# DarioSamo/sm64rt-legacy-renderer

Hardware: AMD Instinct MI355X
Metric: Mrays/s (primary+shadow), sample scene 1080p 1spp (higher is better)
Workload: dtype f32

## Files before the change

sm64rt-legacy-renderer_amd/csrc/kernels.h:

```cpp
#pragma once
#include <hip/hip_runtime.h>
#include "rt64_gpu.h"

#define LBVH_SMALL_MAX 4096u
enum { LBVH_MODE_TRIANGLES = 0, LBVH_MODE_INSTANCES = 1 };

struct LbvhArgs {
    int mode, refit;
    uint32_t n;
    const uint8_t *vertices; uint32_t vertexStride; const uint32_t *indices;
    const GpuInstance *instances;
    GpuNode *nodes;
    GpuTri *tris;
    BlasHeader *header;
    uint32_t *sortedIndex, *morton, *leafParent;
    void *scratch; size_t scratchBytes;
};

size_t lbvh_small_lds_bytes(uint32_t n);
size_t lbvh_large_scratch_bytes(uint32_t n);
hipError_t lbvh_launch(const LbvhArgs &args, hipStream_t stream);
hipError_t lbvh_launch_large(const LbvhArgs &args, hipStream_t stream);
hipError_t lbvh_launch_batch(const LbvhArgs *deviceArgs, uint32_t count, uint32_t maxN, hipStream_t stream);

hipError_t tile_texture_launch(const uint8_t *rgba, uint32_t *tiled, uint32_t width, uint32_t height, hipStream_t stream);
hipError_t bc7_decode_launch(const uint8_t *blocks, uint8_t *rgba, uint32_t width, uint32_t height, hipStream_t stream);

#define RT_CACHE_MAX_WORDS 1536
#define RT_STACK_LDS 24
#define RT_STACK_LDS_CACHED 16
#define RT_STACK_SPILL 84
#define RT_STACK_SPILL_HEADER 2
hipError_t launch_stack_slab_init(uint32_t *slab, size_t lanes, const uint32_t *flagDevicePointer, hipStream_t s);
#define RT_GRID_BLOCKS 2048
#define RT_TIMING_WAVES ((8192u + 8u) * 4u)
#define RT_MAX_BOUNCE_GROUPS 65536u
#define RT_MAX_FRAME_GROUPS 8192u
size_t rt_stack_spill_bytes(int width, int rows);

hipError_t launch_scene_cache_image(const GpuInstance *instances, const uint32_t *tlasIndex, const GpuNode *tlasNodes, uint32_t cacheInstances, void *image, bool blasOnly, hipStream_t s);
hipError_t launch_primary_trace(const FrameParams &P, const ViewImages &I, int32_t *hitInstance, bool klist, hipStream_t s);
hipError_t launch_primary_shade(const FrameParams &P, const ViewImages &I, const int32_t *hitInstance, int cur, bool transparentLighting, bool lean, hipStream_t s);
hipError_t launch_direct(const FrameParams &P, const ViewImages &I, int cur, bool lean, hipStream_t s);
enum { BOUNCE_WALK_PLAIN = 0, BOUNCE_WALK_REFILL = 1, BOUNCE_WALK_SPLIT = 2 };
hipError_t launch_indirect(const FrameParams &P, const ViewImages &I, int cur, bool writeFiltered, bool klist, int walk, unsigned groups, int writeGuide, hipStream_t s);
hipError_t launch_indirect_constant(const FrameParams &P, const ViewImages &I, int cur, hipStream_t s);
hipError_t launch_refraction(const FrameParams &P, const ViewImages &I, bool klist, hipStream_t s);
hipError_t launch_reflection(const FrameParams &P, const ViewImages &I, bool klist, int pass, bool last, int parity, hipStream_t s);
hipError_t launch_gaussian(const uint16_t *in, uint16_t *out, int width, int height, int y0, int y1, hipStream_t s);
hipError_t launch_compose_post(const FrameParams &P, const ViewImages &I, int cur, bool lean, bool writeFinal, hipStream_t s);
hipError_t launch_lean_frame(const FrameParams &P, const ViewImages &I, int32_t *hitInstance, int cur, bool full, int ownedY0, int ownedY1, unsigned maxGroups, bool perWave, hipStream_t s);
hipError_t launch_post_process(const FrameParams &P, const ViewImages &I, hipStream_t s);
hipError_t launch_primary_shade_simple(const FrameParams &P, const ViewImages &I, const int32_t *hitInstance, int cur, bool transparentLighting, bool lean, hipStream_t s);
hipError_t launch_direct_simple(const FrameParams &P, const ViewImages &I, int cur, bool lean, hipStream_t s);
hipError_t launch_indirect_simple(const FrameParams &P, const ViewImages &I, int cur, bool writeFiltered, bool klist, int walk, unsigned groups, int writeGuide, hipStream_t s);
hipError_t launch_refraction_simple(const FrameParams &P, const ViewImages &I, bool klist, hipStream_t s);
// ... 37 lines not shown
```

sm64rt-legacy-renderer_amd/csrc/lbvh.hip:

```cpp
#include <algorithm>
#include "kernels.h"
#include "device_math.h"

#define LBVH_THREADS 1024
#define LBVH_COUNTING_MAX 1024u

namespace {

DEV uint32_t float_to_ordered(float f) { uint32_t u = __float_as_uint(f); return (u & 0x80000000u) ? ~u : (u | 0x80000000u); }
DEV float ordered_to_float(uint32_t u) { return __uint_as_float((u & 0x80000000u) ? (u & 0x7FFFFFFFu) : ~u); }

DEV uint32_t morton30(uint32_t x, uint32_t y, uint32_t z) {
    uint32_t v[3] = { x & 1023u, y & 1023u, z & 1023u };
    uint32_t code = 0;
#pragma unroll
    for (int k = 0; k < 3; k++) {
        uint32_t t = v[k];
        t = (t | (t << 16)) & 0x030000FFu;
        t = (t | (t << 8)) & 0x0300F00Fu;
        t = (t | (t << 4)) & 0x030C30C3u;
        t = (t | (t << 2)) & 0x09249249u;
        code |= t << k;
    }
    return code;
// ... 578 lines not shown

hipError_t lbvh_launch_large(const LbvhArgs &args, hipStream_t stream) {
    if (!args.scratch || args.scratchBytes < lbvh_large_scratch_bytes(args.n)) return hipErrorInvalidValue;
    const uint32_t n = args.n;
    LargeScratch L = carve(args.scratch, n);
    const uint32_t grid = std::min<uint32_t>((n + LG_THREADS - 1) / LG_THREADS, 2048u);
    if (!args.refit) {
        hipLaunchKernelGGL(lg_init_bounds, dim3(1), dim3(64), 0, stream, L.bounds);
        hipLaunchKernelGGL(lg_bounds_kernel, dim3(grid), dim3(LG_THREADS), 0, stream, args, L.bounds);
        hipLaunchKernelGGL(lg_morton_kernel, dim3(grid), dim3(LG_THREADS), 0, stream, args, L.bounds, L.keyA, L.valA);
        uint32_t *kin = L.keyA, *vin = L.valA, *kout = L.keyB, *vout = L.valB;
        for (int shift = 0; shift < 32; shift += 8) {
            hipLaunchKernelGGL(lg_hist_kernel, dim3(L.blocks), dim3(LG_THREADS), 0, stream, kin, n, shift, L.hist, L.blocks);
            hipLaunchKernelGGL(lg_scan_rows_kernel, dim3(256), dim3(LG_THREADS), 0, stream, L.hist, L.blocks);
            hipLaunchKernelGGL(lg_scatter_kernel, dim3(L.blocks), dim3(LG_THREADS), 0, stream, kin, vin, kout, vout, n, shift, L.hist, L.blocks);
            std::swap(kin, kout); std::swap(vin, vout);
        }
        hipLaunchKernelGGL(lg_karras_kernel, dim3(grid), dim3(LG_THREADS), 0, stream, args, kin, vin);
    }
    hipLaunchKernelGGL(lg_leaves_kernel, dim3(grid), dim3(LG_THREADS), 0, stream, args, L.leafBox, L.done);
    uint32_t lists = (n + LG_CHUNK - 1) / LG_CHUNK;
    uint32_t *inList = L.rootList, *inCount = L.rootCount;
    hipLaunchKernelGGL(lg_fit_local_kernel, dim3(lists), dim3(LG_FIT_THREADS), 0, stream, args, L.leafBox, L.nodeBox, inList, inCount);
    for (uint64_t granule = (uint64_t)LG_CHUNK * LG_FAN;; granule *= LG_FAN) {
        const uint32_t groups = (lists + LG_FAN - 1) / LG_FAN;
        uint32_t *outList = inList + (size_t)lists * LG_ROOT_SLOTS, *outCount = inCount + lists;
        hipLaunchKernelGGL(lg_fit_group_kernel, dim3(groups), dim3(1024), 0, stream, args, L.leafBox, L.nodeBox, L.done, inList, inCount, lists,
                           groups == 1 ? 0xFFFFFFFFu : (uint32_t)granule, outList, outCount);
        if (groups == 1) break;
        lists = groups; inList = outList; inCount = outCount;
    }
    return hipGetLastError();
}
```

sm64rt-legacy-renderer_amd/csrc/rt64_gpu.h:

```cpp
#pragma once
#include <stdint.h>
#include "../../include/rt64.h"

#define RT64_LEAF_BIT 0x80000000u
#define RT64_NO_CHILD 0xFFFFFFFFu
#define RT64_MAX_MIPS 16
#define RT64_MAX_LIGHTS 16
#define RT64_MAX_HIT_QUERIES 16

struct alignas(16) GpuNode {
    float lmin[3], lmax[3];
    float rmin[3], rmax[3];
    uint32_t left, right, parent, pad;
};
static_assert(sizeof(GpuNode) == 64, "GpuNode");

struct alignas(16) GpuTri {
    float v0[3]; uint32_t prim;
    float v1[3]; uint32_t pad1;
    float v2[3]; uint32_t pad2;
};
static_assert(sizeof(GpuTri) == 48, "GpuTri");
#define GPU_TRI_FETCH_SLACK_BYTES (sizeof(GpuNode) - sizeof(GpuTri))
static_assert(GPU_TRI_FETCH_SLACK_BYTES == 16 && GPU_TRI_FETCH_SLACK_BYTES <= sizeof(GpuTri), "a triangle is fetched as one node-sized record");
inline size_t gpu_tri_array_bytes(size_t triangles) { return triangles * sizeof(GpuTri) + GPU_TRI_FETCH_SLACK_BYTES; }

struct BlasHeader {
    float bmin[3]; uint32_t count;
    float bmax[3]; uint32_t depth;
};

struct GpuTexture {
    const uint8_t *texels;
    uint32_t width, height, mips, pow2;
    uint32_t mipOffset[RT64_MAX_MIPS];
};

struct GpuCombiner {
    int8_t c[2][4];
    int8_t inputCount, useTex0, useTex1, vertexUV;
    int8_t doSingle[2], doMultiply[2], doMix[2];
    int8_t colorAlphaSame, optAlpha, optTextureEdge, optNoise;
    int16_t vertexSize, normalOffset, uvOffset, inputOffset[4];
};

enum : uint32_t {
    GPU_INST_CULL_DISABLE = 1u << 0,
    GPU_INST_OPAQUE       = 1u << 1,
    GPU_INST_NORMAL_MAP   = 1u << 2,
    GPU_INST_SPECULAR_MAP = 1u << 3,
    GPU_INST_SHADOW_OPAQUE = 1u << 4,
};

struct alignas(16) GpuInstance {
    float objectToWorld[16];
    float objectToWorldNormal[16];
    float objectToWorldPrevious[16];
    float worldToObject[16];
    const GpuNode *nodes;
    const GpuTri *tris;
    const uint8_t *vertices;
    const uint32_t *indices;
    const BlasHeader *header;
    RT64_MATERIAL material;
    GpuCombiner cc;
    int32_t texDiffuse, texNormal, texSpecular;
    uint32_t filter, hAddr, vAddr;
    uint32_t flags;
    uint32_t triCount;
    uint32_t meshVersion;
    uint32_t cacheNodeOffset;
};

struct alignas(16) GpuRasterInstance {
    const uint8_t *vertices;
    const uint32_t *indices;
    uint32_t vertexStride, triCount;
    uint32_t firstTri;
    GpuCombiner cc;
    int32_t texDiffuse;
    uint32_t filter, hAddr, vAddr;
    int32_t scissorRect[4], viewportRect[4];
    uint32_t meshVersion;
    uint32_t texSerial;
};

struct FrameParams {
    float view[16], viewI[16], prevViewI[16], projection[16], projectionI[16], viewProj[16], prevViewProj[16];
    float cameraU[4], cameraV[4], cameraW[4];
    float viewport[4], resolution[4];
    float ambientBaseColor[4], ambientNoGIColor[4], eyeLightDiffuseColor[4], eyeLightSpecularColor[4];
    float skyDiffuseMultiplier[4], skyHSLModifier[4];
    float pixelJitter[2];
    float skyYawOffset, giDiffuseStrength, giSkyStrength, motionBlurStrength;
    int32_t skyPlaneTexIndex;
// ... 33 lines not shown
struct ViewImages {
    uint16_t *viewDirection;
    float *shadingPosition;
    uint16_t *shadingNormal, *shadingSpecular;
    uint8_t *diffuse;
    int32_t *instanceId, *firstInstanceId;
    uint16_t *directLight[2], *indirectLight[2], *filteredDirect[2], *filteredIndirect[2];
    uint16_t *reflection, *refraction, *transparent;
    uint16_t *flow;
    uint8_t *reactiveMask, *lockMask;
    uint16_t *normal[2];
    float *depth[2];
    float *output;
    uint8_t *final;
    uint32_t *primaryHit;
    float *moments[2];
    uint4 *bounceRecords;
    uint32_t *bounceLists, *bounceCounts;
    BounceRadiance *bounceResults;
    uint4 *svgfGuide;
    uint32_t *svgfYoung;
    uint4 *reflState0, *reflState1; uint32_t *reflTag;
    uint32_t *reflectFlags;
    uint4 *klistA;
    uint2 *klistB;
    uint32_t *klistCount;
};

#if defined(__HIPCC__)
#define RT64_HD __host__ __device__ inline
#else
#define RT64_HD inline
#endif
#define RT64_GATHER_MAX_RANKS 64
struct GatherLayout { int height, count, mode; int starts[RT64_GATHER_MAX_RANKS + 1]; };
RT64_HD int gather_band_rows(int height, int count) { return (height + count - 1) / count; }
RT64_HD int gather_row_owner(const GatherLayout &L, int y, int *packed) {
    if (L.count <= 1) { *packed = y; return 0; }
    if (L.mode == 2) { int r = 0; while (r + 1 < L.count && y >= L.starts[r + 1]) r++; *packed = y - L.starts[r]; return r; }
    if (L.mode == 1) { const int b = gather_band_rows(L.height, L.count); *packed = y % b; return y / b; }
    const int strip = y / 16;
    *packed = (strip / L.count) * 16 + (y & 15);
    return strip % L.count;
}
RT64_HD int gather_owned_rows(const GatherLayout &L, int rank) {
    if (L.count <= 1) return L.height;
    if (L.mode == 2) return L.starts[rank + 1] - L.starts[rank];
    if (L.mode == 1) { const int b = gather_band_rows(L.height, L.count), y0 = rank * b, y1 = (rank + 1) * b; return (y1 < L.height ? y1 : L.height) - (y0 < L.height ? y0 : L.height); }
    int rows = 0;
    for (int y = rank * 16; y < L.height; y += L.count * 16) rows += (y + 16 <= L.height ? 16 : L.height - y);
    return rows;
}
RT64_HD int gather_max_owned_rows(const GatherLayout &L) {
    if (L.mode == 2) { int m = 0; for (int r = 0; r < L.count; r++) { const int n = L.starts[r + 1] - L.starts[r]; m = n > m ? n : m; } return m; }
    return L.mode == 1 ? gather_band_rows(L.height, L.count) : (((L.height + 15) / 16 + L.count - 1) / L.count) * 16;
}
RT64_HD GatherLayout gather_layout(int height, int count, int mode) { GatherLayout L; L.height = height; L.count = count < 1 ? 1 : count; L.mode = mode; for (int i = 0; i <= RT64_GATHER_MAX_RANKS; i++) L.starts[i] = 0; return L; }

#define RT_COUNTER_STRIPES 64
enum { CTR_NODES = 0, CTR_TRIS, CTR_PRIMARY, CTR_SHADOW, CTR_INDIRECT, CTR_REFLECTION, CTR_REFRACTION,
       CTR_PASS_BASE,
       CTR_COUNT = CTR_PASS_BASE + 2 * 6 };
enum { PASS_PRIMARY_TRACE = 0, PASS_PRIMARY_SHADE, PASS_DIRECT, PASS_INDIRECT, PASS_REFRACTION, PASS_REFLECTION };
```

sm64rt-legacy-renderer_amd/csrc/rt64_host.cpp:

```cpp
#include <algorithm>
#include <chrono>
#include <cmath>
#include <cstdio>
#include <cstdlib>
#include <cstring>
#include <map>
#include <stdexcept>
#include <string>
#include <vector>

#include "kernels.h"
#include "device_math.h"

#define RT64_EXPORT extern "C" __attribute__((visibility("default")))

namespace rt64 {

static std::string GlobalLastError;

#define HIP_CHECK(call) do { hipError_t e_ = (call); if (e_ != hipSuccess) { \
    char msg_[512]; snprintf(msg_, sizeof(msg_), "HIP call " #call " failed: %s", hipGetErrorString(e_)); throw std::runtime_error(msg_); } } while (0)

template <class T> struct DevArray {
    T *ptr = nullptr; size_t count = 0;
// ... 96 lines not shown

#define RT64_RENDER_STREAMS_MAX 4
#define RT64_LEAN_HOLDOFF_FRAMES 4

struct Options {
    bool countTraversal = false, profilePasses = true, syncPresent = true, alwaysRebuild = false, leanFrames = true, fusedLean = true, foldForeground = true;
    int profileEvery = 1;
    bool leanRecords = false;
    bool framePrologue = true;
    bool hostTlas = true;
    bool simpleKernels = true;
    bool ldsCache = true;
    bool spinPresent = true;
    int perWaveFrame = -1;
    bool tileTiming = false;
    int bounceGroups = -1;
    int bounceSplit = -1;
    int bounceRefill = -1;
    int denoiserMode = 1;
    bool tileOrder = true;
    bool foldCompose = true;
    bool foldVariance = true;
    bool foldGuide = true;
    bool overlapFrames = true;
    bool reflectionEarly = true;
    bool overlapReflection = true;
    bool haloExchange = false;
    bool haloDryRun = false;
    int haloMargin = SVGF_INPUT_HALO_ROWS;
    int maxReflections = 2;
    int giBounces = 1;
    int primarySpp = 1;
    unsigned maxFrameGroups = RT_MAX_FRAME_GROUPS;
};

struct Device {
    int hipDevice = 0;
    hipStream_t stream = nullptr;
    hipStream_t streams[RT64_RENDER_STREAMS_MAX] = {}; int cur = 0, streamCount = 3;
    hipEvent_t streamJoin[RT64_RENDER_STREAMS_MAX] = {};
    bool streamBusy[RT64_RENDER_STREAMS_MAX] = {};
    bool framePure = false, lastFramePure = false;
    void joinStreams() {
        for (int k = 0; k < streamCount; k++) {
            if (k == cur || !streamBusy[k]) continue;
            HIP_CHECK(hipEventRecord(streamJoin[k], streams[k]));
            HIP_CHECK(hipStreamWaitEvent(stream, streamJoin[k], 0));
            streamBusy[k] = false;
        }
    }
    unsigned long long orderedEpoch = 1, seenEpoch[RT64_RENDER_STREAMS_MAX] = {};
    hipEvent_t streamCatchUp = nullptr;
    void noteOrderedWork() { seenEpoch[cur] = ++orderedEpoch; }
    void impure() { framePure = false; joinStreams(); noteOrderedWork(); }
    void enter() { use(); joinStreams(); noteOrderedWork(); lastFramePure = false; }
    void switchStream() {
        const int prev = cur;
        streamBusy[prev] = true; cur = (cur + 1) % streamCount; stream = streams[cur];
        if (seenEpoch[cur] != orderedEpoch) {
            HIP_CHECK(hipEventRecord(streamCatchUp, streams[prev]));
            HIP_CHECK(hipStreamWaitEvent(stream, streamCatchUp, 0));
            seenEpoch[cur] = orderedEpoch;
        }
    }
    int width = 0, height = 0, pendingWidth = 0, pendingHeight = 0;
    int tileY0 = 0, tileY1 = 0; bool tileSet = false;
// ... 64 lines not shown
    }
    std::vector<Mesh *> dirtyMeshes; DevArray<LbvhArgs> buildArgs;
    void flushMeshBuilds();
    void beforeSceneMutation();
    unsigned leanHoldoff = 0;
    void draw(int vsyncInterval, float deltaTimeMs);
    float aspect() const { return (float)width / (float)height; }
    template <class F> void forEachOwnedStrip(F &&f) const {
        for (int y = tileY0 + stripRank * 16; y < tileY1; y += stripCount * 16) f(y, std::min(y + 16, tileY1));
    }
    int ownedRows() const { int r = 0; forEachOwnedStrip([&](int a, int b) { r += b - a; }); return r; }
};

struct Texture {
    Device *device; int width = 0, height = 0, mips = 0;
    DevArray<uint8_t> texels; uint32_t mipOffset[RT64_MAX_MIPS] = {};
    uint8_t minAlpha = 255, maxAlpha = 255;
    int currentIndex = -1;
    uint32_t serial;
    explicit Texture(Device *d) : device(d) { static uint32_t globalTextureSerial = 0; serial = ++globalTextureSerial; }
    void setRGBA8(const void *bytes, int byteCount, int w, int h, int rowPitch);
    void setDDS(const void *bytes, int byteCount);
};

struct Shader {
    Device *device; uint32_t shaderId, filter, hAddr, vAddr; int flags; GpuCombiner cc;
};

struct Mesh {
    Device *device; int flags;
    int vertexCount = 0, vertexStride = 0, indexCount = 0;
    std::vector<uint8_t> hostVertices;
    DevArray<uint8_t> vertices; DevArray<uint32_t> indices;
    DevArray<GpuNode> nodes; DevArray<GpuTri> tris; DevArray<BlasHeader> header;
    DevArray<uint32_t> sortedIndex, morton, leafParent; DevArray<uint8_t> buildScratch;
    uint32_t blasCount = 0;
    float hostBmin[3] = { 0, 0, 0 }, hostBmax[3] = { 0, 0, 0 };
    uint32_t topologyVersion = 0, depth = 255;
    uint32_t treeDepth() const { return blasCount == 0 ? 0u : depth; }
    bool buildPending = false, pendingRefit = false;
    ~Mesh();
    uint32_t version = 0;
    std::map<int, std::pair<float, float>> alphaBounds; uint32_t alphaBoundsVersion = 0;
    Mesh(Device *d, int f) : device(d), flags(f) {}
    void set(const void *vertexArray, int vcount, int vstride, const unsigned int *indexArray, int icount);
    std::pair<float, float> inputAlphaBounds(int offset);
};

struct Instance {
    Scene *scene;
    Mesh *mesh = nullptr; Texture *diffuse = nullptr, *normal = nullptr, *specular = nullptr; Shader *shader = nullptr;
    Mat4 transform = mat_identity(), previousTransform = mat_identity();
    RT64_MATERIAL material = {}; RT64_RECT scissorRect = {}, viewportRect = {}; unsigned int flags = 0;
    explicit Instance(Scene *s);
    ~Instance();
};

struct Scene {
    Device *device; RT64_SCENE_DESC desc = {};
    std::vector<RT64_LIGHT> lights;
    std::vector<Instance *> instances; std::vector<View *> views;
    explicit Scene(Device *d);
    ~Scene();
};

struct RenderInstance { Instance *instance; };
// ... 233 lines not shown
        }
    }
    std::vector<unsigned long long> keys(n);
    float scale[3];
    for (int k = 0; k < 3; k++) { const float ext = smax[k] - smin[k]; scale[k] = ext > 0.0f ? 1024.0f / ext : 0.0f; }
    for (uint32_t t = 0; t < n; t++) {
        uint32_t q[3];
        for (int k = 0; k < 3; k++) {
            const float c = (lo[3 * (size_t)t + k] + hi[3 * (size_t)t + k]) * 0.5f, f = (c - smin[k]) * scale[k];
            q[k] = !(f >= 1.0f) ? 0u : (f >= 1023.0f ? 1023u : (uint32_t)(int)f);
        }
        keys[t] = ((unsigned long long)host_morton30(q[0], q[1], q[2]) << 32) | t;
    }
    std::sort(keys.begin(), keys.end());
    struct Range { uint32_t l, r, d; };
    std::vector<Range> todo; todo.push_back({ 0u, n - 1, 1u });
    uint32_t deepest = 1;
    while (!todo.empty()) {
        const Range g = todo.back(); todo.pop_back();
        deepest = std::max(deepest, g.d);
        const unsigned long long bit = 1ull << (63 - __builtin_clzll(keys[g.l] ^ keys[g.r]));
        uint32_t a = g.l, b = g.r;
        while (a + 1 < b) { const uint32_t m = a + (b - a) / 2; if (keys[m] & bit) b = m; else a = m; }
        if (a > g.l) todo.push_back({ g.l, a, g.d + 1 });
        if (b < g.r) todo.push_back({ b, g.r, g.d + 1 });
    }
    return deepest;
}

void Mesh::set(const void *vertexArray, int vcount, int vstride, const unsigned int *indexArray, int icount) {
    if (!vertexArray || !indexArray || vcount <= 0 || icount <= 0 || vstride < 12) throw std::runtime_error("RT64_SetMesh: invalid arguments.");
    float mn[3] = { INFINITY, INFINITY, INFINITY }, mx[3] = { -INFINITY, -INFINITY, -INFINITY };
    const int usedIndices = (flags & RT64_MESH_RAYTRACE_ENABLED) ? (icount / 3) * 3 : icount;
    for (int i = 0; i < icount; i++) {
        if (indexArray[i] >= (unsigned int)vcount) throw std::runtime_error("RT64_SetMesh: index " + std::to_string(i) + " (" + std::to_string(indexArray[i]) + ") is out of range for " + std::to_string(vcount) + " vertices.");
        if (i < usedIndices) {
            float p[3]; memcpy(p, static_cast<const uint8_t *>(vertexArray) + (size_t)indexArray[i] * vstride, 12);
            for (int k = 0; k < 3; k++) { mn[k] = fminf(mn[k], p[k]); mx[k] = fmaxf(mx[k], p[k]); }
        }
    }
    memcpy(hostBmin, mn, 12); memcpy(hostBmax, mx, 12);
    device->enter();
    if (vertices.ptr) device->beforeSceneMutation();
    const bool sameShape = vertices.ptr && vertexCount == vcount && vertexStride == vstride && indexCount == icount;
    if (buildPending && !pendingRefit && (flags & RT64_MESH_RAYTRACE_ENABLED) && (flags & RT64_MESH_RAYTRACE_UPDATABLE) && sameShape && blasCount == (uint32_t)icount / 3)
        device->flushMeshBuilds();
    const size_t vbytes = (size_t)vcount * vstride, ibytes = (size_t)icount * 4;
    hostVertices.assign(static_cast<const uint8_t *>(vertexArray), static_cast<const uint8_t *>(vertexArray) + vbytes);
    vertices.reserve(vbytes); indices.reserve((size_t)icount);
    uint8_t *stage = static_cast<uint8_t *>(device->ringAlloc(vbytes + ibytes));
    memcpy(stage, vertexArray, vbytes); memcpy(stage + vbytes, indexArray, ibytes);
    HIP_CHECK(hipMemcpyAsync(vertices.ptr, stage, vbytes, hipMemcpyHostToDevice, device->stream));
    HIP_CHECK(hipMemcpyAsync(indices.ptr, stage + vbytes, ibytes, hipMemcpyHostToDevice, device->stream));
    static uint32_t globalMeshVersion = 0;
    vertexCount = vcount; vertexStride = vstride; indexCount = icount; version = ++globalMeshVersion;
    if (flags & RT64_MESH_RAYTRACE_ENABLED) {
        const uint32_t n = (uint32_t)icount / 3;
        if (n == 0) throw std::runtime_error("RT64_SetMesh: a ray-traced mesh needs at least one triangle.");
        const bool refit = (flags & RT64_MESH_RAYTRACE_UPDATABLE) && sameShape && blasCount == n;
        pendingRefit = buildPending ? (pendingRefit && refit) : refit;
        if (!pendingRefit) depth = host_blas_depth(static_cast<const uint8_t *>(vertexArray), (size_t)vstride, indexArray, n);
        nodes.reserve(std::max<size_t>(n - 1, 1)); tris.reserve((gpu_tri_array_bytes(n) + sizeof(GpuTri) - 1) / sizeof(GpuTri)); header.reserve(1);
        if (tris.bytes() < gpu_tri_array_bytes(n)) throw std::runtime_error("RT64_SetMesh: triangle array without its fetch slack.");
        sortedIndex.reserve(n); morton.reserve(n); leafParent.reserve(n);
        if (n > LBVH_SMALL_MAX) buildScratch.reserve(lbvh_large_scratch_bytes(n));
        blasCount = n;
        if (!buildPending) { buildPending = true; device->dirtyMeshes.push_back(this); }
    }
}

Mesh::~Mesh() {
    if (buildPending) { auto &d = device->dirtyMeshes; d.erase(std::remove(d.begin(), d.end(), this), d.end()); }
}

void Device::flushMeshBuilds() {
    if (dirtyMeshes.empty()) return;
    use();
    impure();
    std::vector<LbvhArgs> small; uint32_t maxN = 0;
    for (Mesh *m : dirtyMeshes) {
        LbvhArgs a = {};
        a.mode = LBVH_MODE_TRIANGLES; a.refit = m->pendingRefit ? 1 : 0; a.n = m->blasCount;
        a.vertices = m->vertices.ptr; a.vertexStride = (uint32_t)m->vertexStride; a.indices = m->indices.ptr;
        a.nodes = m->nodes.ptr; a.tris = m->tris.ptr; a.header = m->header.ptr; a.sortedIndex = m->sortedIndex.ptr; a.morton = m->morton.ptr; a.leafParent = m->leafParent.ptr;
        if (a.n > LBVH_SMALL_MAX) { a.scratch = m->buildScratch.ptr; a.scratchBytes = m->buildScratch.bytes(); HIP_CHECK(lbvh_launch_large(a, stream)); }
        else { small.push_back(a); maxN = std::max(maxN, a.n); }
        if (!m->pendingRefit) m->topologyVersion++;
        m->buildPending = false; m->pendingRefit = false;
    }
    dirtyMeshes.clear();
    if (small.size() == 1) HIP_CHECK(lbvh_launch(small[0], stream));
    else if (!small.empty()) {
        const size_t bytes = small.size() * sizeof(LbvhArgs);
        buildArgs.reserve(small.size());
        void *stage = ringAlloc(bytes);
        memcpy(stage, small.data(), bytes);
        HIP_CHECK(hipMemcpyAsync(buildArgs.ptr, stage, bytes, hipMemcpyHostToDevice, stream));
        HIP_CHECK(lbvh_launch_batch(buildArgs.ptr, (uint32_t)small.size(), maxN, stream));
    }
    workSinceMark = true;
}

void Device::beforeSceneMutation() {
    for (Scene *sc : scenes) for (View *v : sc->views) if (v->leanFrame) { v->materialise(); leanHoldoff = RT64_LEAN_HOLDOFF_FRAMES; }
}

std::pair<float, float> Mesh::inputAlphaBounds(int offset) {
    if (alphaBoundsVersion != version) { alphaBounds.clear(); alphaBoundsVersion = version; }
    auto it = alphaBounds.find(offset);
    if (it != alphaBounds.end()) return it->second;
    float mn = INFINITY, mx = -INFINITY;
    for (int v = 0; v < vertexCount; v++) {
        if ((size_t)v * vertexStride + offset + 16 > hostVertices.size()) { mn = NAN; mx = NAN; break; }
        float a; memcpy(&a, hostVertices.data() + (size_t)v * vertexStride + offset + 12, 4);
        if (!(a >= mn)) mn = a;
        if (!(a <= mx)) mx = a;
    }
    return alphaBounds[offset] = std::make_pair(mn, mx);
}


// ... 335 lines not shown
        for (size_t i = 0; i < nInst; i++) deepest = std::max(deepest, rtInstances[i].instance->mesh->treeDepth());
        needSpillSlab = nInst > 0 && std::max<size_t>(nInst - 1, 1) + deepest > RT_STACK_LDS;
    }
    maxDepthBias = nInst ? -INFINITY : 0.0f;
    anyNonOpaque = anyReflection = anyRefraction = anyFog = false;
    simpleFrame = dev->opt.simpleKernels && nInst > 0;
    for (size_t i = 0; i < nInst; i++) {
        Instance *inst = rtInstances[i].instance;
        GpuInstance &g = hInst[i];
        memset(&g, 0, sizeof(g));
        memcpy(g.objectToWorld, inst->transform.m, 64);
        memcpy(g.objectToWorldPrevious, subFrame > 0 ? inst->transform.m : inst->previousTransform.m, 64);
        Mat4 upper = inst->transform;
        upper.m[3] = upper.m[7] = upper.m[11] = 0.0f; upper.m[12] = upper.m[13] = upper.m[14] = 0.0f; upper.m[15] = 1.0f;
        Mat4 nrm = mat_transpose(mat_inverse(upper));
        memcpy(g.objectToWorldNormal, nrm.m, 64);
        Mat4 w2o = mat_inverse(inst->transform);
        memcpy(g.worldToObject, w2o.m, 64);
        Mesh *mesh = inst->mesh;
        g.nodes = mesh->nodes.ptr; g.tris = mesh->tris.ptr; g.vertices = mesh->vertices.ptr; g.indices = mesh->indices.ptr; g.header = mesh->header.ptr;
        g.material = inst->material;
        g.cc = inst->shader->cc;
        g.texDiffuse = g.material.diffuseTexIndex = inst->diffuse->currentIndex;
        g.texNormal = g.material.normalTexIndex = inst->normal ? inst->normal->currentIndex : -1;
        g.texSpecular = g.material.specularTexIndex = inst->specular ? inst->specular->currentIndex : -1;
        g.filter = inst->shader->filter; g.hAddr = inst->shader->hAddr; g.vAddr = inst->shader->vAddr;
        g.flags = 0;
        if (inst->flags & RT64_INSTANCE_DISABLE_BACKFACE_CULLING) g.flags |= GPU_INST_CULL_DISABLE;
        if (instance_is_opaque(inst, g.cc)) g.flags |= GPU_INST_OPAQUE;
        if (inst->shader->flags & RT64_SHADER_NORMAL_MAP_ENABLED) g.flags |= GPU_INST_NORMAL_MAP;
        if (inst->shader->flags & RT64_SHADER_SPECULAR_MAP_ENABLED) g.flags |= GPU_INST_SPECULAR_MAP;
        if (instance_is_shadow_opaque(inst, g.cc)) g.flags |= GPU_INST_SHADOW_OPAQUE;
        else simpleFrame = false;
        g.triCount = mesh->blasCount;
        g.meshVersion = mesh->version;
        g.cacheNodeOffset = cacheWords ? cacheOffset[i] : 0u;
        if (g.cc.vertexSize > mesh->vertexStride) throw std::runtime_error("Instance mesh vertex stride is smaller than the layout its shader reads.");
        maxDepthBias = std::max(maxDepthBias, inst->material.depthBias);
        if (!(g.flags & GPU_INST_OPAQUE)) anyNonOpaque = true;
        if (inst->material.reflectionFactor > 1e-6f) anyReflection = true;
        if (inst->material.refractionFactor > 1e-6f) anyRefraction = true;
        if (inst->material.fogEnabled) anyFog = true;
    }
    for (size_t i = 0; i < nTex; i++) {
        Texture *t = usedTextures[i];
        GpuTexture &g = hTex[i];
        g.texels = t->texels.ptr; g.width = (uint32_t)t->width; g.height = (uint32_t)t->height; g.mips = (uint32_t)t->mips;
        g.pow2 = ((t->width & (t->width - 1)) == 0 && (t->height & (t->height - 1)) == 0) ? 1u : 0u;
        if (!g.pow2) simpleFrame = false;
        memcpy(g.mipOffset, t->mipOffset, sizeof(g.mipOffset));
    }
    if (nLights) memcpy(hLights, scene->lights.data(), lightBytes);
    const size_t tableBytes = instBytes + texBytes + lightBytes;
    const bool sameContent = tab[tabCur].uploadedTables.size() == tableBytes && tableBytes && memcmp(tab[tabCur].uploadedTables.data(), stage, tableBytes) == 0;
    const bool unchanged = sameContent && !dev->opt.alwaysRebuild;
    if (!unchanged) {
        int pick = -1;
        for (int k = 1; k < TABLE_SLOTS && pick < 0; k++) { const int c = (tabCur + k) % TABLE_SLOTS; if (!(tab[c].readers & ~(1u << dev->cur))) pick = c; }
        if (pick < 0) { pick = (tabCur + 1) % TABLE_SLOTS; dev->impure(); }
        tabCur = pick;
        tab[tabCur].readers = 0;
        const uint32_t n = (uint32_t)nInst;
        const bool hostTlas = n >= 1 && n <= RT64_HOST_TLAS_MAX && dev->opt.hostTlas;
        const size_t tlasAt = (tableBytes + 63) & ~(size_t)63, nodeBytes = sizeof(GpuNode) * std::max<size_t>(n ? n - 1 : 0, 1);
        const bool hostCache = hostTlas && cacheWords != 0;
        const size_t cacheAt = (tlasAt + nodeBytes + sizeof(BlasHeader) + 2 * sizeof(uint32_t) * n + 63) & ~(size_t)63, headWords = hostCache ? 4 * (size_t)n + 4 * std::max<size_t>(n - 1, 1) : 0;
// ... 762 lines not shown
}
RT64_EXPORT int RT64_SetDeviceOption(RT64_DEVICE *device, const char *key, double value) {
    Device *d = reinterpret_cast<Device *>(device); if (!d || !key) return 0;
    std::string k = key;
    if (k == "count_traversal") d->opt.countTraversal = value != 0.0;
    else if (k == "profile_passes") d->opt.profilePasses = value != 0.0;
    else if (k == "profile_every") { d->finishStats(); d->opt.profileEvery = std::max(1, (int)value); d->profCounter = 0; }
    else if (k == "sync_present") d->opt.syncPresent = value != 0.0;
    else if (k == "denoiser_mode") d->opt.denoiserMode = (int)value;
    else if (k == "bounce_refill") d->opt.bounceRefill = (int)value;
    else if (k == "overlap_reflection") d->opt.overlapReflection = value != 0.0;
    else if (k == "reflection_early") d->opt.reflectionEarly = value != 0.0;
    else if (k == "overlap_frames") d->opt.overlapFrames = value != 0.0;
    else if (k == "tile_order") d->opt.tileOrder = value != 0.0;
    else if (k == "fold_variance") d->opt.foldVariance = value != 0.0;
    else if (k == "fold_guide") d->opt.foldGuide = value != 0.0;
    else if (k == "fold_compose") d->opt.foldCompose = value != 0.0;
    else if (k == "halo_exchange") d->opt.haloExchange = value != 0.0;
    else if (k == "halo_dry_run") d->opt.haloDryRun = value != 0.0;
    else if (k == "halo_margin") d->opt.haloMargin = std::max((int)value, SVGF_INPUT_HALO_ROWS);
    else if (k == "bounce_split") d->opt.bounceSplit = (int)value;
    else if (k == "bounce_groups") d->opt.bounceGroups = value >= 0.0 && value <= (double)RT_MAX_BOUNCE_GROUPS ? (int)value : -1;
    else if (k == "per_wave_frame") d->opt.perWaveFrame = (int)value;
    else if (k == "tile_timing") d->opt.tileTiming = value != 0.0;
    else if (k == "spin_present") d->opt.spinPresent = value != 0.0;
    else if (k == "lds_cache") d->opt.ldsCache = value != 0.0;
    else if (k == "lean_records") d->opt.leanRecords = value != 0.0;
    else if (k == "host_tlas") d->opt.hostTlas = value != 0.0;
    else if (k == "frame_prologue") d->opt.framePrologue = value != 0.0;
    else if (k == "simple_kernels") d->opt.simpleKernels = value != 0.0;
    else if (k == "reset_accum") { d->finishStats(); d->accum = RT64_FRAME_STATS(); }
    else if (k == "fold_foreground") d->opt.foldForeground = value != 0.0;
    else if (k == "fused_lean") d->opt.fusedLean = value != 0.0;
    else if (k == "lean_frames") d->opt.leanFrames = value != 0.0;
    else if (k == "always_rebuild") d->opt.alwaysRebuild = value != 0.0;
    else if (k == "max_reflections") d->opt.maxReflections = std::max(0, (int)value);
    else if (k == "gi_bounces") { if (value != 1.0 && value != 2.0) return 0; d->opt.giBounces = (int)value; }
    else if (k == "primary_spp") { if (!(value >= 1.0 && value <= 64.0)) return 0; d->opt.primarySpp = (int)value; }
    else if (k == "max_frame_groups") d->opt.maxFrameGroups = value >= 1.0 && value <= (double)RT_MAX_FRAME_GROUPS ? (unsigned)value : RT_MAX_FRAME_GROUPS;
    else return 0;
    return 1;
}
RT64_EXPORT size_t RT64_ReadbackTileTiming(RT64_DEVICE *device, void *dst, size_t dstBytes) {
    RT64_TRY
    Device *d = reinterpret_cast<Device *>(device);
    if (!d || !dst || !d->tileTiming.ptr) throw std::runtime_error("RT64_ReadbackTileTiming: set the device option tile_timing and draw a frame first.");
    d->enter();
    const size_t bytes = std::min(dstBytes, d->tileTiming.bytes());
    HIP_CHECK(hipMemcpyAsync(dst, d->tileTiming.ptr, bytes, hipMemcpyDeviceToHost, d->stream));
    HIP_CHECK(hipStreamSynchronize(d->stream));
    return bytes;
    RT64_CATCH(0)
}
RT64_EXPORT void *RT64_GetDeviceStream(RT64_DEVICE *device) { Device *d = reinterpret_cast<Device *>(device); return d ? d->stream : nullptr; }

RT64_EXPORT RT64_VIEW *RT64_CreateView(RT64_SCENE *scenePtr) {
    RT64_TRY if (!scenePtr) throw std::runtime_error("RT64_CreateView: NULL scene."); return reinterpret_cast<RT64_VIEW *>(new View(reinterpret_cast<Scene *>(scenePtr))); RT64_CATCH(nullptr)
}
RT64_EXPORT void RT64_SetViewPerspective(RT64_VIEW *viewPtr, RT64_MATRIX4 viewMatrix, float fovRadians, float nearDist, float farDist, bool canReproject) {
    View *v = reinterpret_cast<View *>(viewPtr); if (!v) return;
    v->view = mat_from(viewMatrix); v->fov = fovRadians; v->nearDist = nearDist; v->farDist = farDist; v->canReproject = canReproject; v->perspectiveSet = fovRadians > 0.0f;
}
RT64_EXPORT void RT64_SetViewDescription(RT64_VIEW *viewPtr, RT64_VIEW_DESC viewDesc) {
    View *v = reinterpret_cast<View *>(viewPtr); if (!v) return;
    v->resolutionScale = viewDesc.resolutionScale; v->motionBlurStrength = viewDesc.motionBlurStrength; v->maxLights = viewDesc.maxLights;
    v->diSamples = viewDesc.diSamples; v->giSamples = viewDesc.giSamples; v->denoiserEnabled = viewDesc.denoiserEnabled;
// ... 666 lines not shown
```

sm64rt-legacy-renderer_amd/csrc/shade.h:

```cpp
#pragma once
#include "trace.h"


template <bool POW2> DEV int tex_address(int i, int n, uint32_t mode) {
    if (mode == 2) return i < 0 ? 0 : (i >= n ? n - 1 : i);
    if (mode == 1) {
        const int p = 2 * n;
        int j;
        if (POW2) j = i & (p - 1); else { j = i % p; if (j < 0) j += p; }
        return j < n ? j : p - 1 - j;
    }
    if (POW2) return i & (n - 1);
    int j = i % n; if (j < 0) j += n;
    return j;
}

template <class T> DEV T load_const(const T *p) {
    typedef const T __attribute__((address_space(4))) *CP;
    T r; __builtin_memcpy(&r, reinterpret_cast<CP>(reinterpret_cast<uintptr_t>(p)), sizeof(T)); return r;
}
template <class F> DEV void waterfall(uint32_t key, F &&f) {
    bool todo = true;
    while (__ballot(todo) != 0ull) {
        if (todo) {
            const uint32_t k = (uint32_t)__builtin_amdgcn_readfirstlane((int)key);
            if (key == k) {
                f((uint32_t)__builtin_amdgcn_readfirstlane((int)key));
                todo = false;
            }
        }
    }
}

struct TexView { const uint8_t *texels; uint32_t width, height, mips, pow2; const uint32_t *mipOffset; };
struct TexHead { const uint8_t *texels; uint32_t width, height, mips, pow2; };
static_assert(offsetof(GpuTexture, mipOffset) == sizeof(TexHead), "GpuTexture head");
DEV TexView tex_view(const GpuTexture *t) {
    const TexHead h = load_const(reinterpret_cast<const TexHead *>(t));
    TexView v; v.texels = h.texels; v.width = h.width; v.height = h.height; v.mips = h.mips; v.pow2 = h.pow2; v.mipOffset = t->mipOffset;
    return v;
}
DEV TexView tex_view_arg(const GpuTexture __attribute__((address_space(4))) &t) {
    TexView v; v.texels = t.texels; v.width = t.width; v.height = t.height; v.mips = t.mips; v.pow2 = t.pow2; v.mipOffset = nullptr;
    return v;
}

DEV uint32_t tex_mip_offset(const TexView &t, uint32_t level) {
    if (t.mips == 1) return 0;
    return t.mipOffset[level];
}
DEV f4 tex_texel(const TexView &t, uint32_t mipOffset, int x, int y, int w) {
    const uint32_t *base = reinterpret_cast<const uint32_t *>(t.texels) + mipOffset;
    uint32_t v = base[(size_t)y * (size_t)w + (size_t)x];
    const float k = 1.0f / 255.0f;
    return mk4((float)(v & 0xFF) * k, (float)((v >> 8) & 0xFF) * k, (float)((v >> 16) & 0xFF) * k, (float)(v >> 24) * k);
}

template <bool POW2>
DEV f4 tex_sample_level_impl(const TexView &t, float u, float v, uint32_t level, uint32_t filter, uint32_t hAddr, uint32_t vAddr) {
    int w = max((int)(t.width >> level), 1), h = max((int)(t.height >> level), 1);
    const uint32_t mo = tex_mip_offset(t, level);
    if (filter == 0) {
        int x = tex_address<POW2>((int)floorf(u * (float)w), w, hAddr), y = tex_address<POW2>((int)floorf(v * (float)h), h, vAddr);
        return tex_texel(t, mo, x, y, w);
    }
    float x = u * (float)w - 0.5f, y = v * (float)h - 0.5f;
    float x0f = floorf(x), y0f = floorf(y);
    float fx = x - x0f, fy = y - y0f;
    int x0 = tex_address<POW2>((int)x0f, w, hAddr), x1 = tex_address<POW2>((int)x0f + 1, w, hAddr);
    int y0 = tex_address<POW2>((int)y0f, h, vAddr), y1 = tex_address<POW2>((int)y0f + 1, h, vAddr);
    f4 c00 = tex_texel(t, mo, x0, y0, w), c10 = tex_texel(t, mo, x1, y0, w), c01 = tex_texel(t, mo, x0, y1, w), c11 = tex_texel(t, mo, x1, y1, w);
    f4 r;
    { float top = c00.x + fx * (c10.x - c00.x), bot = c01.x + fx * (c11.x - c01.x); r.x = top + fy * (bot - top); }
    { float top = c00.y + fx * (c10.y - c00.y), bot = c01.y + fx * (c11.y - c01.y); r.y = top + fy * (bot - top); }
    { float top = c00.z + fx * (c10.z - c00.z), bot = c01.z + fx * (c11.z - c01.z); r.z = top + fy * (bot - top); }
    { float top = c00.w + fx * (c10.w - c00.w), bot = c01.w + fx * (c11.w - c01.w); r.w = top + fy * (bot - top); }
    return r;
}
DEV f4 tex_sample_level_any(const TexView &t, float u, float v, uint32_t level, uint32_t filter, uint32_t hAddr, uint32_t vAddr) {
    return t.pow2 ? tex_sample_level_impl<true>(t, u, v, level, filter, hAddr, vAddr) : tex_sample_level_impl<false>(t, u, v, level, filter, hAddr, vAddr);
}
DEV f4 tex_sample_level(const TexView &t, float u, float v, uint32_t level, uint32_t filter, uint32_t hAddr, uint32_t vAddr) {
#ifdef RT_ASSUME_SIMPLE
    return tex_sample_level_impl<true>(t, u, v, level, filter, hAddr, vAddr);
#endif
    return t.pow2 ? tex_sample_level_impl<true>(t, u, v, level, filter, hAddr, vAddr) : tex_sample_level_impl<false>(t, u, v, level, filter, hAddr, vAddr);
}

DEV f4 tex_sample_grad(const TexView &t, float u, float v, f2 ddx, f2 ddy, uint32_t filter, uint32_t hAddr, uint32_t vAddr) {
    if (t.mips == 1) return tex_sample_level(t, u, v, 0, filter, hAddr, vAddr);
    float w0 = (float)t.width, h0 = (float)t.height;
    float ax = ddx.x * w0, ay = ddx.y * h0, bx = ddy.x * w0, by = ddy.y * h0;
    float rho = fmaxf(s_sqrt(ax * ax + ay * ay), s_sqrt(bx * bx + by * by));
    float lod = rho > 0.0f ? log2f(rho) : 0.0f;
// ... 126 lines not shown
DEV f3 blue_noise(PRef P, uint32_t px, uint32_t py, uint32_t frame) {
    uint32_t f = frame % 64u;
    uint32_t bx = (f % 8u) * 64u + px % 64u, by = (f / 8u) * 64u + py % 64u;
    uint32_t v = reinterpret_cast<const uint32_t *>(P.blueNoise)[(size_t)by * 512u + bx];
    const float k = 1.0f / 255.0f;
    return mk3((float)(v & 0xFF) * k, (float)((v >> 8) & 0xFF) * k, (float)((v >> 16) & 0xFF) * k);
}


struct RayDiff { f3 dOdx, dOdy, dDdx, dDdy; };

DEV void compute_ray_diffs(f3 nonNormDir, f3 right, f3 up, float vw, float vh, f3 &dDdx, f3 &dDdy) {
    float dd = dot3(nonNormDir, nonNormDir);
    float divd = s_div(2.0f, dd * s_sqrt(dd));
    float dr = dot3(nonNormDir, right), du = dot3(nonNormDir, up);
    dDdx = ((right * dd - nonNormDir * dr) * divd) * s_rcp(vw);
    dDdy = -(((up * dd - nonNormDir * du) * divd) * s_rcp(vh));
}


struct VertexData {
    f3 pos[3], posW[3];
    f2 uv[3];
    f4 input[4];
    f3 vertexPosition, vertexNormal, triangleNormal, vertexTangent, vertexBinormal;
    f2 vertexUV;
};

DEV f3 ld_f3(const uint8_t *p) { const float *f = reinterpret_cast<const float *>(p); return mk3(f[0], f[1], f[2]); }

struct Mat16 { float m[16]; };
struct InstView {
    GpuCombiner cc; RT64_MATERIAL material; Mat16 objectToWorld, objectToWorldNormal, objectToWorldPrevious;
    const uint8_t *vertices; const uint32_t *indices; int32_t texDiffuse, texNormal, texSpecular; uint32_t filter, hAddr, vAddr, flags;
};
struct CombinerWords { uint32_t w[sizeof(GpuCombiner) / 4]; };
static_assert(sizeof(GpuCombiner) % 4 == 0 && offsetof(GpuInstance, cc) % 4 == 0, "GpuCombiner is read as dwords");
struct InstTail { int32_t texDiffuse, texNormal, texSpecular; uint32_t filter, hAddr, vAddr, flags; };
static_assert(offsetof(GpuInstance, flags) - offsetof(GpuInstance, texDiffuse) == offsetof(InstTail, flags), "GpuInstance tail");
DEV InstView inst_view(PRef P, uint32_t instance) {
    const GpuInstance *g = P.instances + instance;
    InstView v;
    const CombinerWords cw = load_const(reinterpret_cast<const CombinerWords *>(&g->cc));
    __builtin_memcpy(&v.cc, &cw, sizeof(v.cc));
    v.material = load_const(&g->material);
    v.objectToWorld = load_const(reinterpret_cast<const Mat16 *>(g->objectToWorld));
    v.objectToWorldNormal = load_const(reinterpret_cast<const Mat16 *>(g->objectToWorldNormal));
    v.objectToWorldPrevious = load_const(reinterpret_cast<const Mat16 *>(g->objectToWorldPrevious));
    v.vertices = load_const(&g->vertices); v.indices = load_const(&g->indices);
    const InstTail tl = load_const(reinterpret_cast<const InstTail *>(&g->texDiffuse));
    v.texDiffuse = tl.texDiffuse; v.texNormal = tl.texNormal; v.texSpecular = tl.texSpecular; v.filter = tl.filter; v.hAddr = tl.hAddr; v.vAddr = tl.vAddr; v.flags = tl.flags;
    return v;
}

DEV void get_vertex_data(const InstView &in, uint32_t prim, const float b[3], bool wantTangent, VertexData &vd) {
    const GpuCombiner &cc = in.cc;
    const uint8_t *vp[3];
    f3 norm[3];
#pragma unroll
    for (int k = 0; k < 3; k++) {
        vp[k] = in.vertices + (size_t)in.indices[3 * prim + k] * (size_t)cc.vertexSize;
        vd.pos[k] = ld_f3(vp[k]);
        vd.posW[k] = mul_point(in.objectToWorld.m, vd.pos[k]);
        norm[k] = ld_f3(vp[k] + cc.normalOffset);
    }
    vd.vertexPosition = (vd.pos[0] * b[0] + vd.pos[1] * b[1]) + vd.pos[2] * b[2];
    f3 vn = (norm[0] * b[0] + norm[1] * b[1]) + norm[2] * b[2];
    f3 tn = -cross3(vd.pos[2] - vd.pos[0], vd.pos[1] - vd.pos[0]);
    vd.vertexNormal = (vn.x != 0.0f || vn.y != 0.0f || vn.z != 0.0f) ? normalize3(vn) : tn;
    vd.triangleNormal = normalize3(mul_vector(in.objectToWorldNormal.m, tn));
    if (cc.vertexUV) {
#pragma unroll
        for (int k = 0; k < 3; k++) { const float *f = reinterpret_cast<const float *>(vp[k] + cc.uvOffset); vd.uv[k].x = f[0]; vd.uv[k].y = f[1]; }
        vd.vertexUV.x = vd.uv[0].x * b[0] + vd.uv[1].x * b[1] + vd.uv[2].x * b[2];
        vd.vertexUV.y = vd.uv[0].y * b[0] + vd.uv[1].y * b[1] + vd.uv[2].y * b[2];
    }
#pragma unroll
    for (int i = 0; i < 4; i++) {
        if (i < cc.inputCount) {
            float r[4];
            const float *f0 = reinterpret_cast<const float *>(vp[0] + cc.inputOffset[i]);
            const float *f1 = reinterpret_cast<const float *>(vp[1] + cc.inputOffset[i]);
            const float *f2p = reinterpret_cast<const float *>(vp[2] + cc.inputOffset[i]);
#pragma unroll
            for (int ch = 0; ch < 3; ch++) r[ch] = f0[ch] * b[0] + f1[ch] * b[1] + f2p[ch] * b[2];
            r[3] = cc.optAlpha ? (f0[3] * b[0] + f1[3] * b[1] + f2p[3] * b[2]) : 1.0f;
            vd.input[i] = mk4(r[0], r[1], r[2], r[3]);
        }
        else vd.input[i] = mk4(0.0f, 0.0f, 0.0f, 0.0f);
    }
    if (wantTangent) {
        float uva = vd.uv[1].x - vd.uv[0].x, uvb = vd.uv[2].x - vd.uv[0].x;
        float uvc = vd.uv[1].y - vd.uv[0].y, uvd = vd.uv[2].y - vd.uv[0].y;
        float uvk = uvb * uvc - uva * uvd;
// ... 342 lines not shown
```

Baseline: 19600.

## De-index triangle vertices into a per-corner stream and compute pow2 mip offsets arithmetically

Adds a GPU gather kernel that, at BLAS build time, expands indexed vertices into a contiguous per-corner buffer. The shader then reads triangle vertices straight from it, skipping the dependent index load. Meshes whose indices are already the identity reuse the vertex buffer directly. Separately, power-of-two textures now compute mip offsets with closed-form arithmetic instead of a table lookup. The cost is extra device memory (budgeted at 64 MiB per mesh), a gather launch on each build, a larger GpuInstance, and a host-side scan for identity indices.

```diff
diff --git a/sm64rt-legacy-renderer_amd/csrc/kernels.h b/sm64rt-legacy-renderer_amd/csrc/kernels.h
--- a/sm64rt-legacy-renderer_amd/csrc/kernels.h
+++ b/sm64rt-legacy-renderer_amd/csrc/kernels.h
@@ -22,6 +22,7 @@
 hipError_t lbvh_launch(const LbvhArgs &args, hipStream_t stream);
 hipError_t lbvh_launch_large(const LbvhArgs &args, hipStream_t stream);
 hipError_t lbvh_launch_batch(const LbvhArgs *deviceArgs, uint32_t count, uint32_t maxN, hipStream_t stream);
+hipError_t corner_gather_launch(const uint8_t *vertices, const uint32_t *indices, uint32_t stride, uint32_t count, uint8_t *corners, hipStream_t stream);
 
 hipError_t tile_texture_launch(const uint8_t *rgba, uint32_t *tiled, uint32_t width, uint32_t height, hipStream_t stream);
 hipError_t bc7_decode_launch(const uint8_t *blocks, uint8_t *rgba, uint32_t width, uint32_t height, hipStream_t stream);
diff --git a/sm64rt-legacy-renderer_amd/csrc/lbvh.hip b/sm64rt-legacy-renderer_amd/csrc/lbvh.hip
--- a/sm64rt-legacy-renderer_amd/csrc/lbvh.hip
+++ b/sm64rt-legacy-renderer_amd/csrc/lbvh.hip
@@ -634,3 +634,32 @@
     }
     return hipGetLastError();
 }
+
+namespace {
+__global__ __launch_bounds__(256) void corner_gather_kernel(const uint8_t *vertices, const uint32_t *indices, uint32_t stride, uint32_t count, uint8_t *corners) {
+    const size_t step = (size_t)gridDim.x * blockDim.x;
+    if ((stride & 3u) == 0) {
+        const uint32_t words = stride >> 2;
+        const size_t total = (size_t)count * words;
+        for (size_t w = (size_t)blockIdx.x * blockDim.x + threadIdx.x; w < total; w += step) {
+            const size_t c = w / words, j = w - c * words;
+            reinterpret_cast<uint32_t *>(corners)[w] = reinterpret_cast<const uint32_t *>(vertices + (size_t)indices[c] * stride)[j];
+        }
+    }
+    else {
+        const size_t total = (size_t)count * stride;
+        for (size_t b = (size_t)blockIdx.x * blockDim.x + threadIdx.x; b < total; b += step) {
+            const size_t c = b / stride, j = b - c * stride;
+            corners[b] = vertices[(size_t)indices[c] * stride + j];
+        }
+    }
+}
+}
+
+hipError_t corner_gather_launch(const uint8_t *vertices, const uint32_t *indices, uint32_t stride, uint32_t count, uint8_t *corners, hipStream_t stream) {
+    if (count == 0) return hipSuccess;
+    const size_t items = (stride & 3u) == 0 ? (size_t)count * (stride >> 2) : (size_t)count * stride;
+    const size_t blocks = (items + 255) / 256;
+    hipLaunchKernelGGL(corner_gather_kernel, dim3((unsigned)(blocks < 4096 ? blocks : 4096)), dim3(256), 0, stream, vertices, indices, stride, count, corners);
+    return hipGetLastError();
+}
diff --git a/sm64rt-legacy-renderer_amd/csrc/rt64_gpu.h b/sm64rt-legacy-renderer_amd/csrc/rt64_gpu.h
--- a/sm64rt-legacy-renderer_amd/csrc/rt64_gpu.h
+++ b/sm64rt-legacy-renderer_amd/csrc/rt64_gpu.h
@@ -50,7 +50,10 @@
     GPU_INST_NORMAL_MAP   = 1u << 2,
     GPU_INST_SPECULAR_MAP = 1u << 3,
     GPU_INST_SHADOW_OPAQUE = 1u << 4,
-};
+    GPU_INST_CORNERS      = 1u << 5,
+};
+
+#define RT64_CORNER_BUDGET_BYTES ((size_t)64 << 20)
 
 struct alignas(16) GpuInstance {
     float objectToWorld[16];
@@ -61,6 +64,7 @@
     const GpuTri *tris;
     const uint8_t *vertices;
     const uint32_t *indices;
+    const uint8_t *corners;
     const BlasHeader *header;
     RT64_MATERIAL material;
     GpuCombiner cc;
@@ -160,6 +164,17 @@
 #else
 #define RT64_HD inline
 #endif
+RT64_HD uint32_t mip_offset_pow2(uint32_t width, uint32_t height, uint32_t level) {
+    const uint32_t a = (uint32_t)__builtin_ctz(width), b = (uint32_t)__builtin_ctz(height);
+    const uint32_t m = a < b ? a : b, M = a < b ? b : a;
+    const uint32_t g = level < m ? level : m;
+    const uint32_t geo = g ? (0x55555555u >> (32 - 2 * g)) << (a + b - 2 * g + 2) : 0u;
+    const uint32_t t = level < M ? level : M;
+    const uint32_t lin = t > g ? (2u << (M - g)) - (2u << (M - t)) : 0u;
+    const uint32_t tail = level > M ? level - M : 0u;
+    return geo + lin + tail;
+}
+
 #define RT64_GATHER_MAX_RANKS 64
 struct GatherLayout { int height, count, mode; int starts[RT64_GATHER_MAX_RANKS + 1]; };
 RT64_HD int gather_band_rows(int height, int count) { return (height + count - 1) / count; }
diff --git a/sm64rt-legacy-renderer_amd/csrc/rt64_host.cpp b/sm64rt-legacy-renderer_amd/csrc/rt64_host.cpp
--- a/sm64rt-legacy-renderer_amd/csrc/rt64_host.cpp
+++ b/sm64rt-legacy-renderer_amd/csrc/rt64_host.cpp
@@ -152,6 +152,8 @@
     int giBounces = 1;
     int primarySpp = 1;
     unsigned maxFrameGroups = RT_MAX_FRAME_GROUPS;
+    bool cornerStream = true;
+    size_t cornerBudget = RT64_CORNER_BUDGET_BYTES;
 };
 
 struct Device {
@@ -282,6 +284,9 @@
     int vertexCount = 0, vertexStride = 0, indexCount = 0;
     std::vector<uint8_t> hostVertices;
     DevArray<uint8_t> vertices; DevArray<uint32_t> indices;
+    DevArray<uint8_t> corners;
+    bool identityIndices = false;
+    bool cornersReady = false;
     DevArray<GpuNode> nodes; DevArray<GpuTri> tris; DevArray<BlasHeader> header;
     DevArray<uint32_t> sortedIndex, morton, leafParent; DevArray<uint8_t> buildScratch;
     uint32_t blasCount = 0;
@@ -581,6 +586,8 @@
     if (!vertexArray || !indexArray || vcount <= 0 || icount <= 0 || vstride < 12) throw std::runtime_error("RT64_SetMesh: invalid arguments.");
     float mn[3] = { INFINITY, INFINITY, INFINITY }, mx[3] = { -INFINITY, -INFINITY, -INFINITY };
     const int usedIndices = (flags & RT64_MESH_RAYTRACE_ENABLED) ? (icount / 3) * 3 : icount;
+    bool identity = true;
+    for (int i = 0; i < usedIndices && identity; i++) identity = indexArray[i] == (unsigned int)i;
     for (int i = 0; i < icount; i++) {
         if (indexArray[i] >= (unsigned int)vcount) throw std::runtime_error("RT64_SetMesh: index " + std::to_string(i) + " (" + std::to_string(indexArray[i]) + ") is out of range for " + std::to_string(vcount) + " vertices.");
         if (i < usedIndices) {
@@ -603,6 +610,7 @@
     HIP_CHECK(hipMemcpyAsync(indices.ptr, stage + vbytes, ibytes, hipMemcpyHostToDevice, device->stream));
     static uint32_t globalMeshVersion = 0;
     vertexCount = vcount; vertexStride = vstride; indexCount = icount; version = ++globalMeshVersion;
+    identityIndices = identity; cornersReady = false;
     if (flags & RT64_MESH_RAYTRACE_ENABLED) {
         const uint32_t n = (uint32_t)icount / 3;
         if (n == 0) throw std::runtime_error("RT64_SetMesh: a ray-traced mesh needs at least one triangle.");
@@ -636,6 +644,13 @@
         else { small.push_back(a); maxN = std::max(maxN, a.n); }
         if (!m->pendingRefit) m->topologyVersion++;
         m->buildPending = false; m->pendingRefit = false;
+        const size_t cornerBytes = (size_t)a.n * 3 * (size_t)m->vertexStride;
+        if (opt.cornerStream && !m->identityIndices && cornerBytes <= opt.cornerBudget) {
+            m->corners.reserve(cornerBytes);
+            HIP_CHECK(corner_gather_launch(m->vertices.ptr, m->indices.ptr, (uint32_t)m->vertexStride, a.n * 3, m->corners.ptr, stream));
+            m->cornersReady = true;
+        }
+        else { m->corners.release(); m->cornersReady = false; }
     }
     dirtyMeshes.clear();
     if (small.size() == 1) HIP_CHECK(lbvh_launch(small[0], stream));
@@ -1037,6 +1052,8 @@
         if (inst->shader->flags & RT64_SHADER_SPECULAR_MAP_ENABLED) g.flags |= GPU_INST_SPECULAR_MAP;
         if (instance_is_shadow_opaque(inst, g.cc)) g.flags |= GPU_INST_SHADOW_OPAQUE;
         else simpleFrame = false;
+        if (dev->opt.cornerStream && mesh->identityIndices) { g.corners = mesh->vertices.ptr; g.flags |= GPU_INST_CORNERS; }
+        else if (dev->opt.cornerStream && mesh->cornersReady && g.cc.vertexSize == mesh->vertexStride) { g.corners = mesh->corners.ptr; g.flags |= GPU_INST_CORNERS; }
         g.triCount = mesh->blasCount;
         g.meshVersion = mesh->version;
         g.cacheNodeOffset = cacheWords ? cacheOffset[i] : 0u;
@@ -1865,6 +1882,8 @@
     else if (k == "reset_accum") { d->finishStats(); d->accum = RT64_FRAME_STATS(); }
     else if (k == "fold_foreground") d->opt.foldForeground = value != 0.0;
     else if (k == "fused_lean") d->opt.fusedLean = value != 0.0;
+    else if (k == "corner_stream") d->opt.cornerStream = value != 0.0;
+    else if (k == "corner_budget") { if (!(value >= 0.0)) return 0; d->opt.cornerBudget = (size_t)value; }
     else if (k == "lean_frames") d->opt.leanFrames = value != 0.0;
     else if (k == "always_rebuild") d->opt.alwaysRebuild = value != 0.0;
     else if (k == "max_reflections") d->opt.maxReflections = std::max(0, (int)value);
diff --git a/sm64rt-legacy-renderer_amd/csrc/shade.h b/sm64rt-legacy-renderer_amd/csrc/shade.h
--- a/sm64rt-legacy-renderer_amd/csrc/shade.h
+++ b/sm64rt-legacy-renderer_amd/csrc/shade.h
@@ -45,8 +45,9 @@
     return v;
 }
 
-DEV uint32_t tex_mip_offset(const TexView &t, uint32_t level) {
+template <bool POW2> DEV uint32_t tex_mip_offset(const TexView &t, uint32_t level) {
     if (t.mips == 1) return 0;
+    if (POW2) return mip_offset_pow2(t.width, t.height, level);
     return t.mipOffset[level];
 }
 DEV f4 tex_texel(const TexView &t, uint32_t mipOffset, int x, int y, int w) {
@@ -59,7 +60,7 @@
 template <bool POW2>
 DEV f4 tex_sample_level_impl(const TexView &t, float u, float v, uint32_t level, uint32_t filter, uint32_t hAddr, uint32_t vAddr) {
     int w = max((int)(t.width >> level), 1), h = max((int)(t.height >> level), 1);
-    const uint32_t mo = tex_mip_offset(t, level);
+    const uint32_t mo = tex_mip_offset<POW2>(t, level);
     if (filter == 0) {
         int x = tex_address<POW2>((int)floorf(u * (float)w), w, hAddr), y = tex_address<POW2>((int)floorf(v * (float)h), h, vAddr);
         return tex_texel(t, mo, x, y, w);
@@ -252,7 +253,7 @@
 struct Mat16 { float m[16]; };
 struct InstView {
     GpuCombiner cc; RT64_MATERIAL material; Mat16 objectToWorld, objectToWorldNormal, objectToWorldPrevious;
-    const uint8_t *vertices; const uint32_t *indices; int32_t texDiffuse, texNormal, texSpecular; uint32_t filter, hAddr, vAddr, flags;
+    const uint8_t *vertices; const uint32_t *indices; const uint8_t *corners; int32_t texDiffuse, texNormal, texSpecular; uint32_t filter, hAddr, vAddr, flags;
 };
 struct CombinerWords { uint32_t w[sizeof(GpuCombiner) / 4]; };
 static_assert(sizeof(GpuCombiner) % 4 == 0 && offsetof(GpuInstance, cc) % 4 == 0, "GpuCombiner is read as dwords");
@@ -267,7 +268,7 @@
     v.objectToWorld = load_const(reinterpret_cast<const Mat16 *>(g->objectToWorld));
     v.objectToWorldNormal = load_const(reinterpret_cast<const Mat16 *>(g->objectToWorldNormal));
     v.objectToWorldPrevious = load_const(reinterpret_cast<const Mat16 *>(g->objectToWorldPrevious));
-    v.vertices = load_const(&g->vertices); v.indices = load_const(&g->indices);
+    v.vertices = load_const(&g->vertices); v.indices = load_const(&g->indices); v.corners = load_const(&g->corners);
     const InstTail tl = load_const(reinterpret_cast<const InstTail *>(&g->texDiffuse));
     v.texDiffuse = tl.texDiffuse; v.texNormal = tl.texNormal; v.texSpecular = tl.texSpecular; v.filter = tl.filter; v.hAddr = tl.hAddr; v.vAddr = tl.vAddr; v.flags = tl.flags;
     return v;
@@ -277,9 +278,16 @@
     const GpuCombiner &cc = in.cc;
     const uint8_t *vp[3];
     f3 norm[3];
+    if (in.flags & GPU_INST_CORNERS) {
+#pragma unroll
+        for (int k = 0; k < 3; k++) vp[k] = in.corners + (size_t)(3 * prim + k) * (size_t)cc.vertexSize;
+    }
+    else {
+#pragma unroll
+        for (int k = 0; k < 3; k++) vp[k] = in.vertices + (size_t)in.indices[3 * prim + k] * (size_t)cc.vertexSize;
+    }
 #pragma unroll
     for (int k = 0; k < 3; k++) {
-        vp[k] = in.vertices + (size_t)in.indices[3 * prim + k] * (size_t)cc.vertexSize;
         vd.pos[k] = ld_f3(vp[k]);
         vd.posW[k] = mul_point(in.objectToWorld.m, vd.pos[k]);
         norm[k] = ld_f3(vp[k] + cc.normalOffset);
```

Measured after the change: 19480, median of 6. Within noise of the previous version (-0.6%).
